# X1X1010/XequiNet

Hardware: AMD Instinct MI355X
Metric: edges/sec + achieved HBM GB/s, energy+force inference, QM9-shape batch (higher is better)
Workload: dtype f32

## Files before the change

include/xeq.h:

```cpp
#ifndef XEQ_H
#define XEQ_H
#include <stdint.h>

#ifdef __cplusplus
extern "C" {
#endif

enum { XEQ_F32 = 0, XEQ_F64 = 1 };
enum { XEQ_RBF_BESSEL = 0, XEQ_RBF_GAUSSIAN = 1, XEQ_RBF_EXPBERN = 2, XEQ_RBF_EXPNORM = 3 };
enum { XEQ_CUTOFF_COSINE = 0, XEQ_CUTOFF_POLYNOMIAL = 1 };
enum {
  XEQ_OK = 0,
  XEQ_ERR_INVALID_ARGUMENT = 1,
  XEQ_ERR_LAUNCH = 2,
  XEQ_ERR_UNSUPPORTED = 3
};

int xeq_version(void);
const char* xeq_last_error(void);
int64_t xeq_launch_count(void);
int64_t xeq_launch_names(int64_t first, char* buf, int64_t cap);


int xeq_csr_rowptr(const int64_t* keys, int64_t n_keys, int64_t n_rows, int32_t* rowptr, void* stream);
// ... 229 lines not shown
int xeq_message_q_wgrad(int dtype, const void* q, const void* basis, int64_t n_edges, int num_basis, int node_dim, const int32_t mul[3],
                        int n_chunks, void* parts, void* stream);

int xeq_message_wq_supported(int num_basis, int node_dim, const int32_t mul[3]);
int xeq_message_wq_fits(int64_t n_nodes, int64_t n_edges, int num_basis, int node_dim, const int32_t mul[3]);
int64_t xeq_message_wq_pcap(int64_t n_nodes, int64_t n_edges);
int xeq_message_wq_waves(void);
int xeq_message_wq_record_floats_for(int num_basis);
int xeq_message_wq_record_floats(void);
int64_t xeq_message_wq_plan_workspace(int64_t n_nodes);
int64_t xeq_message_wq_win_ints(int n_ranges);
int xeq_message_wq_plan(const int32_t* rowptr, const int32_t* perm, const int64_t* owner, const int64_t* gather,
                        int64_t n_nodes, int64_t n_edges, int n_ranges, void* workspace, int64_t workspace_bytes,
                        int32_t* qptr, int32_t* pgath, int32_t* peid, int32_t* qinfo, int32_t* sq, int32_t* sn, int32_t* win,
                        void* stream);
int xeq_edge_basis_wq(const void* vec, int64_t n_nodes, int64_t n_edges, const int32_t* qptr, const int32_t* peid,
                      int rbf_kind, int cutoff_kind, int num_basis, double cutoff, const void* p0, const void* p1,
                      void* basis, void* dbasis, void* stream);
int xeq_message_fwd_wq(int64_t n_nodes, int64_t n_edges, int n_ranges, const int32_t* sq, const int32_t* sn, const int32_t* win,
                       const int32_t* c_rowptr, const int32_t* pgath, const int32_t* qinfo, const void* basis, const void* h,
                       const void* xhat, const void* s_in, const void* x_in, const void* w_rbf, const void* b_rbf,
                       int num_basis, int node_dim, const int32_t mul[3], void* s_out, void* x_out, int xhat_layout,
                       void* stream);
int64_t xeq_message_wq_parts_floats(int64_t n_nodes, int64_t n_edges, const int32_t mul[3]);
#define XEQ_XHAT_HIGHER_L_ZERO 2
#define XEQ_WQ_MIRROR_WALK 4
#define XEQ_WQ_PACKED_WEIGHTS 64
int64_t xeq_message_wq_packed_weight_floats(int num_basis, int node_dim, const int32_t mul[3]);
int xeq_message_wq_pack_weights(const void* w_rbf, const void* b_rbf, int num_basis, int node_dim, const int32_t mul[3], void* packed,
                                void* stream);
// ... 49 lines not shown
                      int64_t n, int node_dim, const int32_t mul[3], int do_norm, const float* w_packed0, const float* w_packed1,
                      const float* w_packed2, int has_bias, double eps, float* cat, int64_t ld_cat, float* p, float* uv_bt,
                      float* stats, void* stream);
int xeq_update_uv_bwd(const float* uv_bt, const float* g_p, const float* g_cat, int64_t ld_cat, const float* g_x_out,
                      const float* g_s_out, const float* a, int64_t ld_a, const float* s, const float* x, const float* stats,
                      const float* ln_w, const float* eq_w, int64_t n, int node_dim, const int32_t mul[3], int do_norm,
                      const float* wt_packed0, const float* wt_packed1, const float* wt_packed2, double eps, float* g_s, float* g_x,
                      float* g_xhat_bt, void* stream);

long long xeq_pack_epoch(void);
void xeq_pack_epoch_bump(void);
int xeq_rowptr_guard(const int32_t* raw, int64_t n_nodes, int64_t capacity, int32_t* rowptr, int32_t* count, void* stream);
int xeq_rowptr_from_degrees(const int32_t* deg, int64_t n_nodes, int64_t capacity, int32_t* rowptr, int32_t* count, int64_t* running_total,
                            void* stream);
int64_t xeq_rowptr_from_degrees_max(void);

int xeq_node_block_supported(int dtype, int node_dim, const int32_t mul[3]);
int xeq_node_block_auto(int64_t n);
int64_t xeq_small_rows_limit(void);
int xeq_node_block_set_waves(int waves);
int64_t xeq_node_block_rows(int64_t n);
int64_t xeq_node_block_fwd_tiles(int with_tail);
int xeq_node_block_pack_fwd(const float* w3, const float* uv0, const float* uv1, const float* uv2, const float* dot, const float* w4,
                            const float* w1_next, const float* w2_next, void* out, void* stream);
int xeq_node_block_fwd(int64_t n, const float* s, const float* x, const float* ln_w, const float* ln_b, const float* eq_w, const float* eq_b,
                       const float* b_uv, const float* b3, const float* b4, double eps, const void* packed, float* p_scratch, float* uv_bt, float* stats,
                       float* pre, float* a, float* ip, float* s_out, float* x_out, const float* ln_w_next, const float* ln_b_next,
                       const float* eq_w_next, const float* eq_b_next, const float* b1_next, const float* b2_next, float* stats_next,
                       float* xhat_next, float* pre_next, float* h_next, void* stream);
int64_t xeq_node_block_bwd_tiles(int with_tail, int with_gx);
// ... 36 lines not shown
```

xequinet_amd/csrc/xeq_common.h:

```cpp
#pragma once
#include <hip/hip_runtime.h>
#include <stdint.h>
#include <stdlib.h>

#include "../../include/xeq.h"

namespace xeq {

void set_error(const char* fmt, ...);
void note_launch(const char* name);

#define XEQ_CHECK_ARG(cond, ...)        \
  do {                                  \
    if (!(cond)) {                      \
      xeq::set_error(__VA_ARGS__);      \
      return XEQ_ERR_INVALID_ARGUMENT;  \
    }                                   \
  } while (0)

#define XEQ_CHECK_LAUNCH(name)                                                   \
  do {                                                                           \
    xeq::note_launch(name);                                                      \
    hipError_t e_ = hipGetLastError();                                           \
    if (e_ != hipSuccess) {                                                      \
// ... 274 lines not shown
    aux[SCAN_WG_THREADS / 64] = run;
  }
  __syncthreads();
  int32_t base = aux[wave] + incl - sum;
  for (int64_t i = i0; i < i1; ++i) {
    const int32_t v = vals[i];
    vals[i] = base;
    base += v;
  }
  const int32_t total = aux[SCAN_WG_THREADS / 64];
  __syncthreads();
  return total;
}
inline size_t wg_scan_lds_bytes(int64_t n) { return sizeof(int32_t) * (size_t)(n + SCAN_WG_THREADS / 64 + 1); }

struct XcdWalk {
  int64_t n_items;
  int chunk;
  int label, slot, n_slots;
  int64_t idx;
  __device__ XcdWalk(int64_t n, int chunk_) : n_items(n), chunk(chunk_) {
    int nb = gridDim.x;
    if (nb >= 8) {
      label = blockIdx.x & 7;
      slot = blockIdx.x >> 3;
      n_slots = (nb - label + 7) >> 3;
    } else {
      label = -1;
      slot = blockIdx.x;
      n_slots = nb;
// ... 28 lines not shown
```

xequinet_amd/csrc/xeq_graph.hip:

```cpp
#include <stdarg.h>
#include <stdio.h>

#include <atomic>
#include <cmath>

#include <hipcub/hipcub.hpp>

#include "xeq_common.h"

namespace xeq {

static thread_local char g_err[512] = "";
void set_error(const char* fmt, ...) {
  va_list ap;
  va_start(ap, fmt);
  vsnprintf(g_err, sizeof(g_err), fmt, ap);
  va_end(ap);
}

static std::atomic<int64_t> g_launches{0};
constexpr int64_t LAUNCH_RING = 8192;
static const char* g_launch_ring[LAUNCH_RING];
void note_launch(const char* name) { g_launch_ring[g_launches.fetch_add(1, std::memory_order_relaxed) & (LAUNCH_RING - 1)] = name; }

// ... 565 lines not shown
__global__ void __launch_bounds__(SCAN_WG_THREADS) k_rowptr_from_degrees(const int32_t* __restrict__ deg, int64_t n, int64_t cap,
                                                                        int32_t* __restrict__ rowptr, int32_t* __restrict__ count,
                                                                        int64_t* __restrict__ running_total) {
  extern __shared__ int32_t scan_lds[];
  const int32_t total = wg_scan_lds([&](int64_t i) { return deg[i]; }, n, scan_lds);
  const bool ok = cap < 0 || (int64_t)total <= cap;
#pragma unroll 4
  for (int64_t i = threadIdx.x; i < n; i += SCAN_WG_THREADS) rowptr[i] = ok ? scan_lds[i] : 0;
  if (threadIdx.x == 0) {
    rowptr[n] = ok ? total : 0;
    if (count) count[0] = total;
    if (running_total) running_total[0] += total;
  }
}

__global__ void k_rowptr_guard(const int32_t* __restrict__ raw, int64_t n, int32_t cap, int32_t* __restrict__ rowptr, int32_t* __restrict__ count) {
  const int64_t i = (int64_t)blockIdx.x * blockDim.x + threadIdx.x;
  if (i > n) return;
  const int32_t total = raw[n];
  if (i == n) count[0] = total;
  rowptr[i] = total > cap ? 0 : raw[i];
}

}

using namespace xeq;

namespace xeq {
template <typename T>
struct CellGeom {
// ... 290 lines not shown
  XEQ_CHECK_ARG((deg || n_nodes == 0) && rowptr && n_nodes >= 0 && capacity < ((int64_t)1 << 31), "xeq_rowptr_from_degrees: bad arguments");
  if (n_nodes > SCAN_WG_MAX_ITEMS) {
    xeq::set_error("xeq_rowptr_from_degrees: %lld nodes (the one-workgroup form takes <= %lld)", (long long)n_nodes, (long long)SCAN_WG_MAX_ITEMS);
    return XEQ_ERR_UNSUPPORTED;
  }
  static const bool attr_ok = hipFuncSetAttribute((const void*)xeq::k_rowptr_from_degrees, hipFuncAttributeMaxDynamicSharedMemorySize,
                                                  (int)wg_scan_lds_bytes(SCAN_WG_MAX_ITEMS)) == hipSuccess;
  XEQ_CHECK_ARG(attr_ok, "xeq_rowptr_from_degrees: cannot reserve %zu bytes of LDS", wg_scan_lds_bytes(SCAN_WG_MAX_ITEMS));
  hipLaunchKernelGGL(xeq::k_rowptr_from_degrees, dim3(1), dim3(SCAN_WG_THREADS), wg_scan_lds_bytes(n_nodes), (hipStream_t)stream, deg, n_nodes,
                     capacity, rowptr, count, running_total);
  XEQ_CHECK_LAUNCH("xeq_rowptr_from_degrees");
  return XEQ_OK;
}
int64_t xeq_rowptr_from_degrees_max(void) { return SCAN_WG_MAX_ITEMS; }

int xeq_pbc_image_counts(int dtype, const void* cell_host, int64_t n_graphs, const int32_t pbc[3], double cutoff, int32_t reps[3]) {
  XEQ_CHECK_ARG(n_graphs >= 1 && cell_host != nullptr && cutoff > 0, "xeq_pbc_image_counts: bad arguments");
  if (dtype == XEQ_F32) xeq::image_counts<float>((const float*)cell_host, n_graphs, pbc, cutoff, reps);
  else if (dtype == XEQ_F64) xeq::image_counts<double>((const double*)cell_host, n_graphs, pbc, cutoff, reps);
  else XEQ_CHECK_ARG(false, "xeq_pbc_image_counts: dtype %d", dtype);
  XEQ_CHECK_ARG(reps[0] <= 64 && reps[1] <= 64 && reps[2] <= 64, "xeq_pbc_image_counts: %d x %d x %d images per axis (degenerate cell?)",
                (int)reps[0], (int)reps[1], (int)reps[2]);
  return XEQ_OK;
}

int xeq_pbc_tables_host(int dtype, const void* cell_host, int64_t n_graphs, const int32_t reps[3], double cutoff, void* out_host,
                        int64_t out_count) {
  XEQ_CHECK_ARG(n_graphs >= 1 && cell_host != nullptr && out_host != nullptr && reps[0] >= 0 && reps[1] >= 0 && reps[2] >= 0,
                "xeq_pbc_tables_host: bad arguments");
  const int64_t nc = (int64_t)(2 * reps[0] + 1) * (2 * reps[1] + 1) * (2 * reps[2] + 1);
// ... 195 lines not shown
```

xequinet_amd/csrc/xeq_message_wq.hip:

```cpp
#include "xeq_common.h"

#include <hipcub/hipcub.hpp>
#include <stdlib.h>

namespace xeq {

typedef float f32x16 __attribute__((ext_vector_type(16)));
typedef float f32x4 __attribute__((ext_vector_type(4)));
typedef int i32x4 __attribute__((ext_vector_type(4)));

typedef __bf16 bf16x8 __attribute__((ext_vector_type(8)));

constexpr bool wq_bftail(int ks) { return ks <= 3; }
constexpr int WQ_TAIL = 24;
constexpr int wq_tailw(int ks) { return ks <= 4 ? 4 : 8; }
constexpr int wq_recf(int ks) { return WQ_TAIL + 2 * wq_tailw(ks) + 8; }
constexpr int wq_yoff(int ks) { return WQ_TAIL + 2 * wq_tailw(ks); }
constexpr int wq_tail_values(int num_basis) { return (num_basis > 16 ? num_basis - 16 : 0) + 1; }
constexpr int wq_ks(int num_basis) {
  return wq_tail_values(num_basis) <= 1 ? 1 : (wq_tail_values(num_basis) <= 5 ? 3 : ((wq_tail_values(num_basis) + 1) / 2 < 4 ? 4 : (wq_tail_values(num_basis) + 1) / 2));
}
constexpr int WQ_REC_MAX = 48;
__device__ __forceinline__ uint32_t wq_bf16_rne(float x) {
  const uint32_t u = __float_as_uint(x);
  return (u + 0x7FFFu + ((u >> 16) & 1u)) >> 16;
}
__device__ __forceinline__ void wq_split3(float x, uint32_t& hi, uint32_t& mid, uint32_t& lo) {
  hi = wq_bf16_rne(x);
  const float r1 = x - __uint_as_float(hi << 16);
  mid = wq_bf16_rne(r1);
  const float r2 = r1 - __uint_as_float(mid << 16);
  lo = wq_bf16_rne(r2);
}
__device__ __forceinline__ int wq_tail_k(int q, int B) { return 16 + q < B ? 16 + q : (16 + q == (B > 16 ? B : 16) ? -1 : -2); }
constexpr uint32_t WQ_FIRST = 1u << 30, WQ_LAST = 1u << 31, WQ_OWNER = (1u << 30) - 1u;
#ifndef XEQ_WQ_WAVES
#define XEQ_WQ_WAVES 4
#endif
constexpr int WQ_WAVES = XEQ_WQ_WAVES;

#ifndef XEQ_WQ_PART_BWD
struct QuadCount {
  const int32_t* rowptr;
  int64_t n;
  __host__ __device__ int32_t operator()(int64_t i) const {
    if (i >= n) return 0;
    const int32_t deg = rowptr[i + 1] - rowptr[i];
    return deg > 0 ? (deg + 3) >> 2 : 1;
  }
};
#ifndef XEQ_WQ_PART_BWD
__global__ void __launch_bounds__(SCAN_WG_THREADS) k_wq_quad_scan(const QuadCount op, int32_t* __restrict__ qptr) {
  extern __shared__ int32_t scan_lds[];
  const int32_t total = wg_scan_lds(op, op.n, scan_lds);
#pragma unroll 4
  for (int64_t i = threadIdx.x; i < op.n; i += SCAN_WG_THREADS) qptr[i] = scan_lds[i];
  if (threadIdx.x == 0) qptr[op.n] = total;
}
#endif

__global__ void k_wq_fill(int64_t E, int64_t n_nodes, const int32_t* __restrict__ rowptr, const int32_t* __restrict__ perm,
                          const int64_t* __restrict__ owner, const int64_t* __restrict__ gather,
                          const int32_t* __restrict__ qptr, int32_t* __restrict__ pgath, int32_t* __restrict__ peid,
// ... 21 lines not shown
  if (k == deg - 1)
    for (int64_t pp = p + 1; pp < 4 * (int64_t)(q0 + nq); ++pp) {
      pgath[pp] = (int32_t)n;
      peid[pp] = -1;
    }
  if ((k & 3) == 0) {
    const int32_t g = k >> 2;
    qinfo[q0 + g] = (uint32_t)n | (g == 0 ? WQ_FIRST : 0u) | (g == nq - 1 ? WQ_LAST : 0u);
  }
}

__global__ void k_wq_streams(const int32_t* __restrict__ qptr, int64_t N, int n_ranges, int32_t* __restrict__ sq,
                             int32_t* __restrict__ sn) {
  const int k = blockIdx.x * blockDim.x + threadIdx.x;
  if (k > 2 * n_ranges) return;
  const int64_t Q = qptr[N];
  if (k == 2 * n_ranges) {
    sq[k] = (int32_t)Q;
    sn[k] = (int32_t)N;
    return;
  }
  const int64_t target = (int64_t)k * Q / (2 * n_ranges);
  int64_t lo = 0, hi = N;
  while (lo < hi) {
    const int64_t mid = (lo + hi) >> 1;
    if (qptr[mid] >= target) hi = mid;
    else lo = mid + 1;
  }
  sq[k] = qptr[lo];
  sn[k] = (int32_t)lo;
}

__global__ void k_wq_windows(const int32_t* __restrict__ sq, const int32_t* __restrict__ pgath, int n_ranges, int n_steps, int mult,
                             int32_t* __restrict__ win) {
  const int step = blockIdx.x, lane = threadIdx.x;
  if (step >= n_steps) return;
  const int k0 = min(2 * WQ_WAVES * mult * step, 2 * n_ranges), k1 = min(k0 + 2 * WQ_WAVES * mult, 2 * n_ranges);
  const int64_t p0 = 4 * (int64_t)sq[k0], p1 = 4 * (int64_t)sq[k1];
  int lo = 0x7fffffff, hi = -1;
  for (int64_t p = p0 + lane; p < p1; p += 64) {
    const int g = pgath[p];
    lo = g < lo ? g : lo;
    hi = g > hi ? g : hi;
  }
#pragma unroll
// ... 1546 lines not shown
    size_t temp = (size_t)workspace_bytes;
    if (hipcub::DeviceScan::ExclusiveSum(workspace, temp, it, qptr, (int)(n_nodes + 1), (hipStream_t)stream) != hipSuccess) {
      xeq::set_error("xeq_message_wq_plan: scan failed");
      return XEQ_ERR_LAUNCH;
    }
  }
  if (n_edges + n_nodes > 0) {
    hipLaunchKernelGGL(k_wq_fill, dim3((unsigned)((n_edges + n_nodes + 255) / 256)), dim3(256), 0, (hipStream_t)stream, n_edges, n_nodes,
                       rowptr, perm, owner, gather, (const int32_t*)qptr, pgath, peid, (uint32_t*)qinfo);
    XEQ_CHECK_LAUNCH("xeq_message_wq_plan (fill)");
  }
  const int n = 2 * n_ranges + 1;
  hipLaunchKernelGGL(k_wq_streams, dim3((unsigned)((n + 255) / 256)), dim3(256), 0, (hipStream_t)stream, (const int32_t*)qptr,
                     n_nodes, n_ranges, sq, sn);
  XEQ_CHECK_LAUNCH("xeq_message_wq_plan (streams)");
  const int n_steps = wq_class_steps(n_ranges, 1);
  hipLaunchKernelGGL(k_wq_windows, dim3((unsigned)n_steps), dim3(64), 0, (hipStream_t)stream, (const int32_t*)sq,
                     (const int32_t*)pgath, n_ranges, n_steps, 1, win);
  XEQ_CHECK_LAUNCH("xeq_message_wq_plan (windows)");
  const int mlong = wq_long_mult(n_edges, n_ranges);
  if (mlong > 1) {
    const int n_long = wq_class_steps(n_ranges, mlong);
    hipLaunchKernelGGL(k_wq_windows, dim3((unsigned)n_long), dim3(64), 0, (hipStream_t)stream, (const int32_t*)sq,
                       (const int32_t*)pgath, n_ranges, n_long, mlong, win + 2 * n_steps);
    XEQ_CHECK_LAUNCH("xeq_message_wq_plan (windows, long class)");
  }
  return XEQ_OK;
}

int64_t xeq_message_wq_win_ints(int n_ranges) {
  return 2 * ((int64_t)wq_class_steps(n_ranges, 1) + (int64_t)wq_class_steps(n_ranges, 2) + 1);
}

int xeq_edge_basis_wq(const void* vec, int64_t n_nodes, int64_t n_edges, const int32_t* qptr, const int32_t* peid,
                      int rbf_kind, int cutoff_kind, int num_basis, double cutoff, const void* p0, const void* p1,
                      void* basis, void* dbasis, void* stream) {
  XEQ_CHECK_ARG(n_edges >= 0 && n_nodes >= 0 && num_basis >= 1 && num_basis <= 31 && cutoff > 0, "xeq_edge_basis_wq: bad sizes");
  XEQ_CHECK_ARG(rbf_kind >= XEQ_RBF_BESSEL && rbf_kind <= XEQ_RBF_EXPNORM, "xeq_edge_basis_wq: rbf kernel %d is not implemented", rbf_kind);
  XEQ_CHECK_ARG(rbf_kind == XEQ_RBF_BESSEL || p1 != nullptr, "xeq_edge_basis_wq: this radial basis needs its second parameter array (std / logc / mu)");
// ... 166 lines not shown
```

xequinet_amd/lib.py:

```python
from __future__ import annotations

import ctypes
import os
from ctypes import c_char_p, c_double, c_int, c_int32, c_int64, c_void_p
from typing import Optional

import torch

_HERE = os.path.dirname(os.path.abspath(__file__))
LIB_PATH = os.environ.get("XEQ_LIB_PATH") or os.path.join(_HERE, "libxeq_hip.so")

XEQ_F32, XEQ_F64 = 0, 1
COPY_MANY_MAX = 16
SB_ACCUM_VEC = 16
XHAT_HIGHER_L_ZERO = 2
SB_Y0_ZERO = 8
SB_Q_ACCUMULATE = 16
SB_NO_GY = 32
WQ_MIRROR_WALK = 4
WQ_PACKED_WEIGHTS = 64
WQ_MAX_PART_SETS = 8
RBF_KINDS = {"bessel": 0, "gaussian": 1, "expbern": 2, "expnorm": 3}
CUTOFF_KINDS = {"cosine": 0, "polynomial": 1}

_P = c_void_p
# ... 39 lines not shown
    "xeq_eqln_bwd": [c_int, _P, _P, _P, c_int64, _I3, c_double, _P, _P],
    "xeq_segment_sum": [c_int, _P, _P, c_int64, c_int64, _P, _P],
    "xeq_linear_supported": [c_int, c_int, c_int],
    "xeq_mfma_order_probe": [_P, _P, _P, _P],
    "xeq_linear_fwd": [_P, c_int64, c_int64, c_int, _P, _P, c_int, c_int, c_int, _P, _P, c_int64, _P],
    "xeq_head_dot": [_P, c_int64, c_int, _P, _P, _P, _P],
    "xeq_head_bwd_hidden": [_P, c_int64, c_int, _P, _P, _P, _P],
    "xeq_head_supported": [c_int, c_int, c_int],
    "xeq_head_fwd": [_P, c_int64, c_int64, c_int, c_int, _P, _P, _P, _P, _P, _P, _P],
    "xeq_head_bwd": [_P, c_int64, c_int, _P, c_int64, _P, c_int64, _P, _P, _P],
    "xeq_electronic_supported": [c_int, c_int],
    "xeq_electronic_fwd": [c_int, _P, c_int64, c_int64, c_int, _P, c_int64, _P, _P, _P, _P, _P, _P, _P, _P, _P],
    "xeq_first_block_front": [_P, c_int, c_int64, c_int64, _P, _P, _P, c_int, c_int, c_int64, _P, _P, _P, _P],
    "xeq_rowptr_from_degrees": [_P, c_int64, c_int64, _P, _P, _P, _P],
    "xeq_rowptr_from_degrees_max": [],
    "xeq_wgrad_chunks": [c_int64, c_int, c_int],
    "xeq_wgrad": [_P, c_int64, _P, c_int64, c_int64, c_int, c_int, c_int, c_int, _P, _P],
    "xeq_load_padded_batch": [c_int, _P, _P, _P, _P, c_int64, c_int64, c_int64, c_int64, c_double, c_double, _P, _P, _P, _P, _P],
    "xeq_load_padded_batch_z64": [c_int, _P, _P, _P, _P, c_int64, c_int64, c_int64, c_int64, c_double, c_double, _P, _P, _P, _P, _P],
    "xeq_load_padded_shard": [c_int, _P, _P, c_int, _P, _P, c_int64, c_int64, c_int64, c_int64, c_int64, c_int64, c_double, c_double, _P, _P, _P, _P, _P],
    "xeq_copy_many": [c_int, ctypes.POINTER(c_void_p), ctypes.POINTER(c_void_p), ctypes.POINTER(c_int64), _P],
    "xeq_compare_many": [c_int, ctypes.POINTER(c_void_p), ctypes.POINTER(c_void_p), ctypes.POINTER(c_int64), ctypes.c_int32, _P, _P],
    "xeq_tensor_product_path": [c_int, _P, _P, c_int64, c_int, c_int, c_int, c_int, c_int, c_int, c_int, c_int, c_int, c_int, c_int,
                                c_int, c_int, _P, _P, c_int64, c_double, _P, _P],
    "xeq_tensor_product": [c_int, _P, _P, c_int64, c_int, c_int, c_int, c_int, ctypes.POINTER(ctypes.c_int32), _P, ctypes.POINTER(ctypes.c_int32),
                           c_int, _P, c_int64, ctypes.POINTER(ctypes.c_int32), ctypes.POINTER(c_double), _P, _P],
    "xeq_tensor_product_wgrad": [c_int, _P, _P, _P, c_int64, c_int, c_int, c_int, c_int, ctypes.POINTER(ctypes.c_int32), _P,
                                 ctypes.POINTER(ctypes.c_int32), ctypes.POINTER(ctypes.c_int32), ctypes.POINTER(ctypes.c_int32), c_int,
                                 ctypes.POINTER(c_double), c_int, _P, _P],
    "xeq_tensor_product_wgrad_chunks": [c_int64],
# ... 207 lines not shown
```

xequinet_amd/ops.py:

```python
from __future__ import annotations

import ctypes
from typing import Optional, Tuple

import torch
from torch.autograd import Function
from torch.autograd.function import once_differentiable

from . import lib
from .lib import call, dtype_code, mul3, ptr, require_hip, stream


class _KernelTimer:

    def __init__(self) -> None:
        self.enabled = False
        self.events = {}

    def reset(self, enabled: bool) -> None:
        self.enabled = enabled
        self.events = {}

    def launch(self, name: str, *args, label: Optional[str] = None) -> None:
        if not self.enabled:
# ... 108 lines not shown
            assert center_sorted and c_rowptr is not None
        if exact_mirror:
            rev = torch.empty(E, dtype=torch.int32, device=edge_index.device)
            call("xeq_reverse_edge_map", lib.ptr(edge_index), E, self.n_nodes, lib.ptr(self.c_rowptr), lib.ptr(rev), stream())
            self.mirror_map = rev
            self._n_view = (self.c_rowptr, rev)
        elif periodic_mirror:
            off = cell_offsets.contiguous()
            assert off.shape == (E, 3) and off.is_floating_point()
            rev = torch.empty(E, dtype=torch.int32, device=edge_index.device)
            call("xeq_reverse_edge_map_pbc", dtype_code(off), lib.ptr(edge_index), lib.ptr(off), E, self.n_nodes, lib.ptr(self.c_rowptr),
                 lib.ptr(rev), stream())
            self.mirror_map = rev
        else:
            self._sorted_neighbor_view()

    def _sorted_neighbor_view(self):
        if self._n_view is None:
            nbr = self.edge_index[1]
            if self._capacity_form:
                self._n_view = csr_by_key(nbr, self.n_nodes, n_valid=self.c_rowptr[self.n_nodes:])
            else:
                self._n_view = csr_by_key(nbr, self.n_nodes)
        return self._n_view

    @property
    def n_rowptr(self) -> torch.Tensor:
        return self._sorted_neighbor_view()[0]

    @property
# ... 113 lines not shown
    deg = torch.empty(N, dtype=torch.int32, device=dev)
    rowptr = torch.empty(N + 1, dtype=torch.int32, device=dev)
    dt = dtype_code(pos)
    call("xeq_radius_graph_count", dt, ptr(pos), ptr(ptr_), G, N, float(cutoff), ptr(deg), stream())
    count = torch.empty(1, dtype=torch.int32, device=dev)
    if N <= _scan_one_launch_max():
        call("xeq_rowptr_from_degrees", ptr(deg), N, cap, ptr(rowptr), ptr(count), ptr(running_total), stream())
    else:
        raw = torch.empty(N + 1, dtype=torch.int32, device=dev)
        _exclusive_scan(deg, N, raw)
        call("xeq_rowptr_guard", ptr(raw), N, cap, ptr(rowptr), ptr(count), stream())
        if running_total is not None:
            running_total.add_(count)
    call("xeq_radius_graph_fill", dt, ptr(pos), ptr(ptr_), G, N, float(cutoff), ptr(rowptr), cap, ptr(edge_index), stream())
    return rowptr, count


def radius_graph_pbc_raw(pos_wrap, ptr_, img, cells, shift, cutoff, prune=None):
    require_hip(pos_wrap, ptr_, img, cells, shift)
    pos_wrap, img, cells, shift = (t.contiguous() for t in (pos_wrap, img, cells, shift))
    if prune is not None and len(prune) == 4:
        recip, thr, reps, nbins = prune
        recip, thr = recip.to(pos_wrap.dtype).contiguous(), thr.to(pos_wrap.dtype).contiguous()
        nbins = nbins.to(torch.int32).contiguous()
        ptr_ = ptr_.to(torch.int64).contiguous()
        N, G, n_cells = pos_wrap.shape[0], ptr_.numel() - 1, cells.shape[0]
        dev, dt = pos_wrap.device, dtype_code(pos_wrap)
        per_graph = nbins.prod(dim=1)
        bin_base = torch.zeros(G + 1, dtype=torch.int32, device=dev)
        bin_base[1:] = torch.cumsum(per_graph, 0)
# ... 65 lines not shown
    _exclusive_scan(deg, N, rowptr)
    count = rowptr[N:].clone()
    rowptr.clamp_(max=cap)
    call("xeq_radius_graph_pbc_fill_pruned", dt, ptr(pos_wrap), ptr(ptr_), G, N, ptr(img), ptr(cells), ptr(shift), n_cells,
         float(cutoff), ptr(recip), ptr(thr), mul3(reps), ptr(rowptr), cap, ptr(edge_index), ptr(cell_offsets), stream())
    return rowptr, count


class EdgeVectors(Function):

    @staticmethod
    def forward(ctx, pos, graph: EdgeGraph, cell, cell_offsets, batch, strain=None, graph_ptr=None):
        require_hip(pos)
        pos_c = pos.contiguous()
        E = graph.n_edges
        vec = torch.empty((E, 3), dtype=pos.dtype, device=pos.device)
        dist = torch.empty((E,), dtype=pos.dtype, device=pos.device)
        cell, cell_offsets, batch = _c(cell), _c(cell_offsets), _c(batch)
        call("xeq_edge_vectors_fwd", dtype_code(pos), ptr(pos_c), ptr(graph.edge_index), E, ptr(cell), ptr(cell_offsets),
             ptr(batch), ptr(vec), ptr(dist), stream())
        graph._basis = None
        for plan in (graph._wq or {}).values():
            plan["records"] = None
        ctx.graph = graph
        ctx.graph_ptr = graph_ptr
        ctx.n_graphs = None if strain is None else strain.shape[0]
        ctx.save_for_backward(vec, dist)
        ctx.set_materialize_grads(False)
        return vec, dist

    @staticmethod
    @once_differentiable
    def backward(ctx, g_vec, g_dist):
        vec, dist = ctx.saved_tensors
        graph = ctx.graph
# ... 739 lines not shown
```

xequinet_amd/runtime.py:

```python
from __future__ import annotations

from collections import OrderedDict
from typing import Dict, Optional

import torch

from . import keys, lib, ops


class _Captured:
    def __init__(self) -> None:
        self.graph: Optional[torch.cuda.CUDAGraph] = None
        self.inputs: Dict[str, torch.Tensor] = {}
        self.edge_graph: Optional[ops.EdgeGraph] = None
        self.derived_batch = False
        self.outputs: Dict[str, torch.Tensor] = {}
        self.static: Dict[str, object] = {}
        self.graph_same: Optional[torch.cuda.CUDAGraph] = None
        self.outputs_same: Dict[str, torch.Tensor] = {}


def refuse_electronic(model, who: str) -> None:
    m = model
    while not isinstance(m, torch.nn.Module) and hasattr(m, "model"):
# ... 183 lines not shown
    mods = getattr(net, "mods", None)
    emb = mods["embedding"] if (mods is not None and "embedding" in mods) else None
    if emb is None or not hasattr(emb, "node_irreps"):
        return
    zero = getattr(step, "_zero_x", None)
    if zero is None:
        zero = step._zero_x = torch.zeros((step.n_atoms, emb.node_irreps.dim), dtype=step.pos.dtype, device=step.pos.device)
    data[ZERO_EQUIVARIANT] = zero


class GraphedStep:

    PAD_SPACING = 100.0

    def __init__(self, model: torch.nn.Module, capacity, cutoff: Optional[float] = None, compute_forces: bool = True, warmup: int = 2,
                 device=None, dtype=None) -> None:
        refuse_electronic(model, "GraphedStep")
        self.model = model
        self.n_atoms, self.n_graphs, self.n_edges = (int(c) for c in capacity)
        self.n_graphs += 1
        self.cutoff = float(model.cutoff_radius if cutoff is None else cutoff)
        self.compute_forces = compute_forces
        p = next(model.parameters())
        dev = p.device if device is None else torch.device(device)
        dt = p.dtype if dtype is None else dtype
        N, G, E = self.n_atoms, self.n_graphs, self.n_edges
        self.pos = torch.zeros((N, 3), dtype=dt, device=dev)
        self.z = torch.zeros(N, dtype=torch.int32, device=dev)
        self.ptr = torch.zeros(G + 1, dtype=torch.int64, device=dev)
        self.batch = torch.zeros(N, dtype=torch.int64, device=dev)
        self.edge_index = torch.zeros((2, max(E, 1)), dtype=torch.int64, device=dev)
        self.graph: Optional[torch.cuda.CUDAGraph] = None
        self.outputs: Dict[str, torch.Tensor] = {}
        self.rowptr: Optional[torch.Tensor] = None
        self.warmup = warmup
        self.captures = 0
        self._param_state = None
        self.edge_total = torch.zeros(1, dtype=torch.int64, device=self.pos.device)

    def overflowed(self) -> bool:
        return bool(self.outputs) and int(self.outputs["n_edges"].item()) > self.n_edges

    def _step(self) -> Dict[str, torch.Tensor]:
        rowptr, count = ops.radius_graph_capacity(self.pos, self.ptr, self.cutoff, self.edge_index, running_total=self.edge_total)
        eg = ops.EdgeGraph(self.edge_index, self.n_atoms, center_sorted=True, ptr=self.ptr, c_rowptr=rowptr, symmetric=True)
        data = {keys.POSITIONS: self.pos.detach(), keys.ATOMIC_NUMBERS: self.z, keys.EDGE_INDEX: self.edge_index, keys.BATCH: self.batch,
                keys.BATCH_PTR: self.ptr, keys.EDGE_GRAPH: eg}
        _offer_zero_start(self, data)
        with torch.enable_grad():
            out = self.model(data, compute_forces=self.compute_forces, compute_virial=False)
        res = {k: v.detach() for k, v in out.items() if isinstance(v, torch.Tensor)}
        res["n_edges"] = count
        return res

    def _load_shard(self, pos: torch.Tensor, atomic_numbers: torch.Tensor, ptr: torch.Tensor, batch: torch.Tensor, a: int, b: int, g0: int,
                    g1: int) -> None:
        from .lib import call, dtype_code
        from ctypes import c_void_p

        n, g = b - a, g1 - g0
# ... 512 lines not shown
```

Before: 181.0 million.

## Merge radius-graph fill with message work-quad plan and edge vectors

Adds a single-workgroup front scan that produces rowptr, quad pointers and stream boundaries together. It also adds a fill kernel that writes edge indices, edge vectors, distances, reverse map and the work-quad gather tables in one pass. The graphed step uses this merged path by default when every message layer picks the wq implementation, and the edge-vector op reuses the precomputed vectors. This removes separate plan, reverse-map and edge-vector kernels from the graph front, at the cost of an O(i) inner loop per hit for computing reverse indices.

```diff
diff --git a/include/xeq.h b/include/xeq.h
--- a/include/xeq.h
+++ b/include/xeq.h
@@ -267,6 +267,7 @@
                         int64_t n_nodes, int64_t n_edges, int n_ranges, void* workspace, int64_t workspace_bytes,
                         int32_t* qptr, int32_t* pgath, int32_t* peid, int32_t* qinfo, int32_t* sq, int32_t* sn, int32_t* win,
                         void* stream);
+int xeq_message_wq_windows(const int32_t* sq, const int32_t* pgath, int64_t n_edges, int n_ranges, int32_t* win, void* stream);
 int xeq_edge_basis_wq(const void* vec, int64_t n_nodes, int64_t n_edges, const int32_t* qptr, const int32_t* peid,
                       int rbf_kind, int cutoff_kind, int num_basis, double cutoff, const void* p0, const void* p1,
                       void* basis, void* dbasis, void* stream);
@@ -346,6 +347,11 @@
 int xeq_rowptr_from_degrees(const int32_t* deg, int64_t n_nodes, int64_t capacity, int32_t* rowptr, int32_t* count, int64_t* running_total,
                             void* stream);
 int64_t xeq_rowptr_from_degrees_max(void);
+int xeq_front_scan(const int32_t* deg, int64_t n_nodes, int64_t capacity, int n_ranges, int32_t* rowptr, int32_t* count,
+                   int64_t* running_total, int32_t* qptr, int32_t* sq, int32_t* sn, void* stream);
+int xeq_radius_graph_fill_plan(int dtype, const void* pos, const int64_t* ptr, int64_t n_graphs, int64_t n_nodes, double cutoff,
+                               const int32_t* rowptr, const int32_t* count, int64_t n_edges, const int32_t* qptr, int64_t* edge_index,
+                               void* vec, void* dist, int32_t* rev, int32_t* pgath, int32_t* peid, int32_t* qinfo, void* stream);
 
 int xeq_node_block_supported(int dtype, int node_dim, const int32_t mul[3]);
 int xeq_node_block_auto(int64_t n);
diff --git a/xequinet_amd/csrc/xeq_common.h b/xequinet_amd/csrc/xeq_common.h
--- a/xequinet_amd/csrc/xeq_common.h
+++ b/xequinet_amd/csrc/xeq_common.h
@@ -312,6 +312,27 @@
 }
 inline size_t wg_scan_lds_bytes(int64_t n) { return sizeof(int32_t) * (size_t)(n + SCAN_WG_THREADS / 64 + 1); }
 
+__host__ __device__ __forceinline__ int32_t wq_quads_of_degree(int32_t deg) { return deg > 0 ? (deg + 3) >> 2 : 1; }
+constexpr uint32_t WQ_FIRST = 1u << 30, WQ_LAST = 1u << 31, WQ_OWNER = (1u << 30) - 1u;
+template <typename QP>
+__device__ __forceinline__ void wq_stream_boundary(const QP& qptr, int64_t N, int64_t Q, int k, int n_ranges, int32_t* __restrict__ sq,
+                                                   int32_t* __restrict__ sn) {
+  if (k == 2 * n_ranges) {
+    sq[k] = (int32_t)Q;
+    sn[k] = (int32_t)N;
+    return;
+  }
+  const int64_t target = (int64_t)k * Q / (2 * n_ranges);
+  int64_t lo = 0, hi = N;
+  while (lo < hi) {
+    const int64_t mid = (lo + hi) >> 1;
+    if (qptr(mid) >= target) hi = mid;
+    else lo = mid + 1;
+  }
+  sq[k] = qptr(lo);
+  sn[k] = (int32_t)lo;
+}
+
 struct XcdWalk {
   int64_t n_items;
   int chunk;
diff --git a/xequinet_amd/csrc/xeq_graph.hip b/xequinet_amd/csrc/xeq_graph.hip
--- a/xequinet_amd/csrc/xeq_graph.hip
+++ b/xequinet_amd/csrc/xeq_graph.hip
@@ -603,6 +603,101 @@
   }
 }
 
+__global__ void __launch_bounds__(SCAN_WG_THREADS) k_front_scan(const int32_t* __restrict__ deg, int64_t n, int64_t cap, int n_ranges,
+                                                               int32_t* __restrict__ rowptr, int32_t* __restrict__ count,
+                                                               int64_t* __restrict__ running_total, int32_t* __restrict__ qptr,
+                                                               int32_t* __restrict__ sq, int32_t* __restrict__ sn) {
+  extern __shared__ int32_t scan_lds[];
+  const int32_t total = wg_scan_lds([&](int64_t i) { return deg[i]; }, n, scan_lds);
+  const bool ok = cap < 0 || (int64_t)total <= cap;
+#pragma unroll 4
+  for (int64_t i = threadIdx.x; i < n; i += SCAN_WG_THREADS) rowptr[i] = ok ? scan_lds[i] : 0;
+  if (threadIdx.x == 0) {
+    rowptr[n] = ok ? total : 0;
+    if (count) count[0] = total;
+    if (running_total) running_total[0] += total;
+  }
+  __syncthreads();
+  const int32_t quads = wg_scan_lds([&](int64_t i) { return wq_quads_of_degree(ok ? deg[i] : 0); }, n, scan_lds);
+#pragma unroll 4
+  for (int64_t i = threadIdx.x; i < n; i += SCAN_WG_THREADS) qptr[i] = scan_lds[i];
+  if (threadIdx.x == 0) qptr[n] = quads;
+  for (int k = threadIdx.x; k <= 2 * n_ranges; k += SCAN_WG_THREADS)
+    wq_stream_boundary([&](int64_t m) { return m < n ? scan_lds[m] : quads; }, n, quads, k, n_ranges, sq, sn);
+}
+
+template <typename T> __device__ __forceinline__ T edge_length(T v0, T v1, T v2);
+template <> __device__ __forceinline__ float edge_length<float>(float v0, float v1, float v2) {
+  return sqrt_<float>(__fmaf_rn(v2, v2, __fmaf_rn(v0, v0, __fmul_rn(v1, v1))));
+}
+template <> __device__ __forceinline__ double edge_length<double>(double v0, double v1, double v2) {
+  return sqrt_<double>(__fma_rn(v2, v2, __fma_rn(v0, v0, __dmul_rn(v1, v1))));
+}
+
+template <typename T>
+__global__ void k_radius_graph_fill_plan(const T* __restrict__ pos, const int64_t* __restrict__ ptr, int64_t n_graphs, int64_t n_nodes, T r2,
+                                         const int32_t* __restrict__ rowptr, const int32_t* __restrict__ count, int64_t n_edges,
+                                         const int32_t* __restrict__ qptr, int64_t* __restrict__ edge_index, T* __restrict__ vec,
+                                         T* __restrict__ dist, int32_t* __restrict__ rev, int32_t* __restrict__ pgath,
+                                         int32_t* __restrict__ peid, uint32_t* __restrict__ qinfo) {
+  const int lane = threadIdx.x & 63;
+  const int64_t i = ((int64_t)blockIdx.x * blockDim.x + threadIdx.x) >> 6;
+  if (i >= n_nodes) return;
+  const bool fits = (int64_t)count[0] <= n_edges;
+  const int64_t q0 = qptr[i];
+  int32_t deg = 0;
+  if (fits) {
+    const int64_t g = graph_of(ptr, n_graphs, i);
+    const int64_t a = ptr[g], b = ptr[g + 1];
+    const T xi = pos[3 * i], yi = pos[3 * i + 1], zi = pos[3 * i + 2];
+    const int64_t r0 = rowptr[i];
+    int64_t w = r0;
+    for (int64_t j0 = a; j0 < b; j0 += 64) {
+      const int64_t j = j0 + lane;
+      bool hit = false;
+      T xj = T(0), yj = T(0), zj = T(0), dx = T(0), dy = T(0), dz = T(0);
+      if (j < b) {
+        xj = pos[3 * j], yj = pos[3 * j + 1], zj = pos[3 * j + 2];
+        dx = sub_rn<T>(xi, xj), dy = sub_rn<T>(yi, yj), dz = sub_rn<T>(zi, zj);
+        T d2 = add_rn<T>(add_rn<T>(mul_rn<T>(dx, dx), mul_rn<T>(dy, dy)), mul_rn<T>(dz, dz));
+        hit = d2 < r2 && j != i;
+      }
+      const unsigned long long m = __ballot(hit);
+      if (m != 0ull) {
+        int32_t below = 0;
+        for (int64_t k = a; k < i; ++k) {
+          const T ex = sub_rn<T>(xj, pos[3 * k]), ey = sub_rn<T>(yj, pos[3 * k + 1]), ez = sub_rn<T>(zj, pos[3 * k + 2]);
+          const T e2 = add_rn<T>(add_rn<T>(mul_rn<T>(ex, ex), mul_rn<T>(ey, ey)), mul_rn<T>(ez, ez));
+          below += (e2 < r2 && k != j) ? 1 : 0;
+        }
+        if (hit) {
+          const int64_t p = w + __popcll(m & ((1ull << lane) - 1ull));
+          if (p < n_edges) {
+            edge_index[p] = i;
+            edge_index[n_edges + p] = j;
+            vec[3 * p] = dx;
+            vec[3 * p + 1] = dy;
+            vec[3 * p + 2] = dz;
+            if (dist) dist[p] = edge_length<T>(dx, dy, dz);
+            rev[p] = rowptr[j] + below;
+            const int64_t s = 4 * q0 + (p - r0);
+            pgath[s] = (int32_t)j;
+            peid[s] = (int32_t)p;
+          }
+        }
+      }
+      w += __popcll(m);
+    }
+    deg = (int32_t)(w - r0);
+  }
+  const int32_t nq = wq_quads_of_degree(deg);
+  if (lane < 4 * nq - deg) {
+    pgath[4 * q0 + deg + lane] = (int32_t)i;
+    peid[4 * q0 + deg + lane] = -1;
+  }
+  for (int32_t q = lane; q < nq; q += 64) qinfo[q0 + q] = (uint32_t)i | (q == 0 ? WQ_FIRST : 0u) | (q == nq - 1 ? WQ_LAST : 0u);
+}
+
 __global__ void k_rowptr_guard(const int32_t* __restrict__ raw, int64_t n, int32_t cap, int32_t* __restrict__ rowptr, int32_t* __restrict__ count) {
   const int64_t i = (int64_t)blockIdx.x * blockDim.x + threadIdx.x;
   if (i > n) return;
@@ -923,6 +1018,42 @@
 }
 int64_t xeq_rowptr_from_degrees_max(void) { return SCAN_WG_MAX_ITEMS; }
 
+int xeq_front_scan(const int32_t* deg, int64_t n_nodes, int64_t capacity, int n_ranges, int32_t* rowptr, int32_t* count,
+                   int64_t* running_total, int32_t* qptr, int32_t* sq, int32_t* sn, void* stream) {
+  XEQ_CHECK_ARG((deg || n_nodes == 0) && rowptr && qptr && sq && sn && n_nodes >= 0 && n_ranges >= 1 && capacity < ((int64_t)1 << 31),
+                "xeq_front_scan: bad arguments");
+  if (n_nodes > SCAN_WG_MAX_ITEMS) {
+    xeq::set_error("xeq_front_scan: %lld nodes (the one-workgroup form takes <= %lld)", (long long)n_nodes, (long long)SCAN_WG_MAX_ITEMS);
+    return XEQ_ERR_UNSUPPORTED;
+  }
+  static const bool attr_ok = hipFuncSetAttribute((const void*)xeq::k_front_scan, hipFuncAttributeMaxDynamicSharedMemorySize,
+                                                  (int)wg_scan_lds_bytes(SCAN_WG_MAX_ITEMS)) == hipSuccess;
+  XEQ_CHECK_ARG(attr_ok, "xeq_front_scan: cannot reserve %zu bytes of LDS", wg_scan_lds_bytes(SCAN_WG_MAX_ITEMS));
+  hipLaunchKernelGGL(xeq::k_front_scan, dim3(1), dim3(SCAN_WG_THREADS), wg_scan_lds_bytes(n_nodes), (hipStream_t)stream, deg, n_nodes,
+                     capacity, n_ranges, rowptr, count, running_total, qptr, sq, sn);
+  XEQ_CHECK_LAUNCH("xeq_front_scan");
+  return XEQ_OK;
+}
+
+int xeq_radius_graph_fill_plan(int dtype, const void* pos, const int64_t* ptr, int64_t n_graphs, int64_t n_nodes, double cutoff,
+                               const int32_t* rowptr, const int32_t* count, int64_t n_edges, const int32_t* qptr, int64_t* edge_index,
+                               void* vec, void* dist, int32_t* rev, int32_t* pgath, int32_t* peid, int32_t* qinfo, void* stream) {
+  XEQ_CHECK_ARG(n_graphs >= 0 && n_nodes >= 0 && n_edges >= 0 && n_edges < ((int64_t)1 << 31) && n_nodes < ((int64_t)1 << 30),
+                "xeq_radius_graph_fill_plan: bad sizes");
+  if (n_nodes == 0) return XEQ_OK;
+  XEQ_CHECK_ARG(n_graphs > 0, "xeq_radius_graph_fill_plan: nodes without graphs");
+  XEQ_CHECK_ARG(pos && ptr && rowptr && count && qptr && edge_index && vec && rev && pgath && peid && qinfo,
+                "xeq_radius_graph_fill_plan: NULL argument");
+  XEQ_DISPATCH_FLOAT(dtype, {
+    T rc = (T)cutoff;
+    hipLaunchKernelGGL((k_radius_graph_fill_plan<T>), dim3((unsigned)((n_nodes + 3) / 4)), dim3(256), 0, (hipStream_t)stream,
+                       (const T*)pos, ptr, n_graphs, n_nodes, rc * rc, rowptr, count, n_edges, qptr, edge_index, (T*)vec, (T*)dist, rev,
+                       pgath, peid, (uint32_t*)qinfo);
+  });
+  XEQ_CHECK_LAUNCH("xeq_radius_graph_fill_plan");
+  return XEQ_OK;
+}
+
 int xeq_pbc_image_counts(int dtype, const void* cell_host, int64_t n_graphs, const int32_t pbc[3], double cutoff, int32_t reps[3]) {
   XEQ_CHECK_ARG(n_graphs >= 1 && cell_host != nullptr && cutoff > 0, "xeq_pbc_image_counts: bad arguments");
   if (dtype == XEQ_F32) xeq::image_counts<float>((const float*)cell_host, n_graphs, pbc, cutoff, reps);
diff --git a/xequinet_amd/csrc/xeq_message_wq.hip b/xequinet_amd/csrc/xeq_message_wq.hip
--- a/xequinet_amd/csrc/xeq_message_wq.hip
+++ b/xequinet_amd/csrc/xeq_message_wq.hip
@@ -33,7 +33,6 @@
   lo = wq_bf16_rne(r2);
 }
 __device__ __forceinline__ int wq_tail_k(int q, int B) { return 16 + q < B ? 16 + q : (16 + q == (B > 16 ? B : 16) ? -1 : -2); }
-constexpr uint32_t WQ_FIRST = 1u << 30, WQ_LAST = 1u << 31, WQ_OWNER = (1u << 30) - 1u;
 #ifndef XEQ_WQ_WAVES
 #define XEQ_WQ_WAVES 4
 #endif
@@ -45,8 +44,7 @@
   int64_t n;
   __host__ __device__ int32_t operator()(int64_t i) const {
     if (i >= n) return 0;
-    const int32_t deg = rowptr[i + 1] - rowptr[i];
-    return deg > 0 ? (deg + 3) >> 2 : 1;
+    return wq_quads_of_degree(rowptr[i + 1] - rowptr[i]);
   }
 };
 #ifndef XEQ_WQ_PART_BWD
@@ -98,21 +96,7 @@
                              int32_t* __restrict__ sn) {
   const int k = blockIdx.x * blockDim.x + threadIdx.x;
   if (k > 2 * n_ranges) return;
-  const int64_t Q = qptr[N];
-  if (k == 2 * n_ranges) {
-    sq[k] = (int32_t)Q;
-    sn[k] = (int32_t)N;
-    return;
-  }
-  const int64_t target = (int64_t)k * Q / (2 * n_ranges);
-  int64_t lo = 0, hi = N;
-  while (lo < hi) {
-    const int64_t mid = (lo + hi) >> 1;
-    if (qptr[mid] >= target) hi = mid;
-    else lo = mid + 1;
-  }
-  sq[k] = qptr[lo];
-  sn[k] = (int32_t)lo;
+  wq_stream_boundary([&](int64_t m) { return qptr[m]; }, N, qptr[N], k, n_ranges, sq, sn);
 }
 
 __global__ void k_wq_windows(const int32_t* __restrict__ sq, const int32_t* __restrict__ pgath, int n_ranges, int n_steps, int mult,
@@ -1689,15 +1673,19 @@
   hipLaunchKernelGGL(k_wq_streams, dim3((unsigned)((n + 255) / 256)), dim3(256), 0, (hipStream_t)stream, (const int32_t*)qptr,
                      n_nodes, n_ranges, sq, sn);
   XEQ_CHECK_LAUNCH("xeq_message_wq_plan (streams)");
+  return xeq_message_wq_windows(sq, pgath, n_edges, n_ranges, win, stream);
+}
+
+int xeq_message_wq_windows(const int32_t* sq, const int32_t* pgath, int64_t n_edges, int n_ranges, int32_t* win, void* stream) {
+  XEQ_CHECK_ARG(sq && pgath && win && n_edges >= 0 && n_ranges >= 1, "xeq_message_wq_windows: bad arguments");
   const int n_steps = wq_class_steps(n_ranges, 1);
-  hipLaunchKernelGGL(k_wq_windows, dim3((unsigned)n_steps), dim3(64), 0, (hipStream_t)stream, (const int32_t*)sq,
-                     (const int32_t*)pgath, n_ranges, n_steps, 1, win);
+  hipLaunchKernelGGL(k_wq_windows, dim3((unsigned)n_steps), dim3(64), 0, (hipStream_t)stream, sq, pgath, n_ranges, n_steps, 1, win);
   XEQ_CHECK_LAUNCH("xeq_message_wq_plan (windows)");
   const int mlong = wq_long_mult(n_edges, n_ranges);
   if (mlong > 1) {
     const int n_long = wq_class_steps(n_ranges, mlong);
-    hipLaunchKernelGGL(k_wq_windows, dim3((unsigned)n_long), dim3(64), 0, (hipStream_t)stream, (const int32_t*)sq,
-                       (const int32_t*)pgath, n_ranges, n_long, mlong, win + 2 * n_steps);
+    hipLaunchKernelGGL(k_wq_windows, dim3((unsigned)n_long), dim3(64), 0, (hipStream_t)stream, sq, pgath, n_ranges, n_long, mlong,
+                       win + 2 * n_steps);
     XEQ_CHECK_LAUNCH("xeq_message_wq_plan (windows, long class)");
   }
   return XEQ_OK;
diff --git a/xequinet_amd/lib.py b/xequinet_amd/lib.py
--- a/xequinet_amd/lib.py
+++ b/xequinet_amd/lib.py
@@ -9,6 +9,8 @@
 
 _HERE = os.path.dirname(os.path.abspath(__file__))
 LIB_PATH = os.environ.get("XEQ_LIB_PATH") or os.path.join(_HERE, "libxeq_hip.so")
+
+FRONT_MERGED = os.environ.get("XEQ_FRONT_SEPARATE", "0") in ("", "0")
 
 XEQ_F32, XEQ_F64 = 0, 1
 COPY_MANY_MAX = 16
@@ -78,6 +80,9 @@
     "xeq_first_block_front": [_P, c_int, c_int64, c_int64, _P, _P, _P, c_int, c_int, c_int64, _P, _P, _P, _P],
     "xeq_rowptr_from_degrees": [_P, c_int64, c_int64, _P, _P, _P, _P],
     "xeq_rowptr_from_degrees_max": [],
+    "xeq_front_scan": [_P, c_int64, c_int64, c_int, _P, _P, _P, _P, _P, _P, _P],
+    "xeq_radius_graph_fill_plan": [c_int, _P, _P, c_int64, c_int64, c_double, _P, _P, c_int64, _P, _P, _P, _P, _P, _P, _P, _P, _P],
+    "xeq_message_wq_windows": [_P, _P, c_int64, c_int, _P, _P],
     "xeq_wgrad_chunks": [c_int64, c_int, c_int],
     "xeq_wgrad": [_P, c_int64, _P, c_int64, c_int64, c_int, c_int, c_int, c_int, _P, _P],
     "xeq_load_padded_batch": [c_int, _P, _P, _P, _P, c_int64, c_int64, c_int64, c_int64, c_double, c_double, _P, _P, _P, _P, _P],
diff --git a/xequinet_amd/ops.py b/xequinet_amd/ops.py
--- a/xequinet_amd/ops.py
+++ b/xequinet_amd/ops.py
@@ -146,6 +146,20 @@
             self.mirror_map = rev
         else:
             self._sorted_neighbor_view()
+
+    @classmethod
+    def prebuilt(cls, edge_index: torch.Tensor, n_nodes: int, ptr: Optional[torch.Tensor], c_rowptr: torch.Tensor, mirror_map: torch.Tensor,
+                 plan_key, plan, vec: torch.Tensor, dist: torch.Tensor, pos: torch.Tensor) -> "EdgeGraph":
+        g = cls.__new__(cls)
+        g.ptr, g._wq, g._basis = ptr, {plan_key: plan}, None
+        g.edge_index, g.n_nodes, g.n_edges = edge_index, int(n_nodes), int(edge_index.shape[1])
+        g.c_perm, g.c_rowptr = None, c_rowptr
+        g.mirror_walk, g.periodic, g.cell_offsets = True, False, None
+        g.mirror_map = mirror_map
+        g.edge_count_on_device, g._capacity_form = False, False
+        g._n_view = (c_rowptr, mirror_map)
+        g._edge_vectors = (pos.data_ptr(), vec, dist)
+        return g
 
     def _sorted_neighbor_view(self):
         if self._n_view is None:
@@ -289,6 +303,34 @@
             running_total.add_(count)
     call("xeq_radius_graph_fill", dt, ptr(pos), ptr(ptr_), G, N, float(cutoff), ptr(rowptr), cap, ptr(edge_index), stream())
     return rowptr, count
+
+
+def radius_graph_capacity_plan(pos: torch.Tensor, ptr_: torch.Tensor, cutoff: float, edge_index: torch.Tensor,
+                               running_total: Optional[torch.Tensor] = None):
+    require_hip(pos, ptr_, edge_index)
+    pos = pos.detach().contiguous()
+    ptr_ = ptr_.to(torch.int64).contiguous()
+    assert edge_index.dim() == 2 and edge_index.shape[0] == 2 and edge_index.dtype == torch.int64 and edge_index.is_contiguous()
+    N, G, cap = pos.shape[0], ptr_.numel() - 1, int(edge_index.shape[1])
+    assert pos.dtype == torch.float32 and 0 < N <= _scan_one_launch_max()
+    dev, dt, L = pos.device, dtype_code(pos), lib.load()
+    eps = _wq_edges_per_stream(cap, N)
+    n_ranges = max(1, -(-cap // (2 * eps)))
+    pcap = int(L.xeq_message_wq_pcap(N, cap))
+    i32 = lambda n: torch.empty(max(int(n), 1), dtype=torch.int32, device=dev)
+    deg, rowptr, count, rev = i32(N), i32(N + 1), i32(1), i32(cap)
+    plan = {"reverse": False, "n_ranges": n_ranges, "pcap": pcap, "qptr": i32(N + 1), "pgath": i32(pcap), "peid": i32(pcap),
+            "qinfo": i32(pcap // 4), "sq": i32(2 * n_ranges + 1), "sn": i32(2 * n_ranges + 1),
+            "win": i32(int(L.xeq_message_wq_win_ints(n_ranges))), "work": None, "records": None, "rowptr": rowptr}
+    vec = torch.empty((cap, 3), dtype=pos.dtype, device=dev)
+    dist = torch.empty((cap,), dtype=pos.dtype, device=dev)
+    call("xeq_radius_graph_count", dt, ptr(pos), ptr(ptr_), G, N, float(cutoff), ptr(deg), stream())
+    call("xeq_front_scan", ptr(deg), N, cap, n_ranges, ptr(rowptr), ptr(count), ptr(running_total), ptr(plan["qptr"]), ptr(plan["sq"]),
+         ptr(plan["sn"]), stream())
+    call("xeq_radius_graph_fill_plan", dt, ptr(pos), ptr(ptr_), G, N, float(cutoff), ptr(rowptr), ptr(count), cap, ptr(plan["qptr"]),
+         ptr(edge_index), ptr(vec), ptr(dist), ptr(rev), ptr(plan["pgath"]), ptr(plan["peid"]), ptr(plan["qinfo"]), stream())
+    call("xeq_message_wq_windows", ptr(plan["sq"]), ptr(plan["pgath"]), cap, n_ranges, ptr(plan["win"]), stream())
+    return EdgeGraph.prebuilt(edge_index, N, ptr_, rowptr, rev, (False, int(eps)), plan, vec, dist, pos), count
 
 
 def radius_graph_pbc_raw(pos_wrap, ptr_, img, cells, shift, cutoff, prune=None):
@@ -384,11 +426,15 @@
         require_hip(pos)
         pos_c = pos.contiguous()
         E = graph.n_edges
-        vec = torch.empty((E, 3), dtype=pos.dtype, device=pos.device)
-        dist = torch.empty((E,), dtype=pos.dtype, device=pos.device)
-        cell, cell_offsets, batch = _c(cell), _c(cell_offsets), _c(batch)
-        call("xeq_edge_vectors_fwd", dtype_code(pos), ptr(pos_c), ptr(graph.edge_index), E, ptr(cell), ptr(cell_offsets),
-             ptr(batch), ptr(vec), ptr(dist), stream())
+        ready, graph._edge_vectors = getattr(graph, "_edge_vectors", None), None
+        if ready is not None and cell is None and ready[0] == pos_c.data_ptr():
+            vec, dist = ready[1], ready[2]
+        else:
+            vec = torch.empty((E, 3), dtype=pos.dtype, device=pos.device)
+            dist = torch.empty((E,), dtype=pos.dtype, device=pos.device)
+            cell, cell_offsets, batch = _c(cell), _c(cell_offsets), _c(batch)
+            call("xeq_edge_vectors_fwd", dtype_code(pos), ptr(pos_c), ptr(graph.edge_index), E, ptr(cell), ptr(cell_offsets),
+                 ptr(batch), ptr(vec), ptr(dist), stream())
         graph._basis = None
         for plan in (graph._wq or {}).values():
             plan["records"] = None
diff --git a/xequinet_amd/runtime.py b/xequinet_amd/runtime.py
--- a/xequinet_amd/runtime.py
+++ b/xequinet_amd/runtime.py
@@ -221,7 +221,7 @@
     PAD_SPACING = 100.0
 
     def __init__(self, model: torch.nn.Module, capacity, cutoff: Optional[float] = None, compute_forces: bool = True, warmup: int = 2,
-                 device=None, dtype=None) -> None:
+                 device=None, dtype=None, merged_front: Optional[bool] = None) -> None:
         refuse_electronic(model, "GraphedStep")
         self.model = model
         self.n_atoms, self.n_graphs, self.n_edges = (int(c) for c in capacity)
@@ -244,13 +244,28 @@
         self.captures = 0
         self._param_state = None
         self.edge_total = torch.zeros(1, dtype=torch.int64, device=self.pos.device)
+        self.merged_front = (lib.FRONT_MERGED if merged_front is None else bool(merged_front)) and self._takes_merged_front()
+
+    def _takes_merged_front(self) -> bool:
+        from .nn.xpainn import XPainnMessage
+
+        net = self.model
+        while not isinstance(net, torch.nn.Module) and hasattr(net, "model"):
+            net = net.model
+        msgs = [m for m in net.modules() if isinstance(m, XPainnMessage)] if isinstance(net, torch.nn.Module) else []
+        if not msgs or self.pos.dtype != torch.float32 or not self.pos.is_cuda or not 0 < self.n_atoms <= ops._scan_one_launch_max():
+            return False
+        return all(ops.select_message_impl(self.pos.dtype, self.n_atoms, max(self.n_edges, 1), m.num_basis, m.node_dim, m._mul) == "wq" for m in msgs)
 
     def overflowed(self) -> bool:
         return bool(self.outputs) and int(self.outputs["n_edges"].item()) > self.n_edges
 
     def _step(self) -> Dict[str, torch.Tensor]:
-        rowptr, count = ops.radius_graph_capacity(self.pos, self.ptr, self.cutoff, self.edge_index, running_total=self.edge_total)
-        eg = ops.EdgeGraph(self.edge_index, self.n_atoms, center_sorted=True, ptr=self.ptr, c_rowptr=rowptr, symmetric=True)
+        if self.merged_front:
+            eg, count = ops.radius_graph_capacity_plan(self.pos, self.ptr, self.cutoff, self.edge_index, running_total=self.edge_total)
+        else:
+            rowptr, count = ops.radius_graph_capacity(self.pos, self.ptr, self.cutoff, self.edge_index, running_total=self.edge_total)
+            eg = ops.EdgeGraph(self.edge_index, self.n_atoms, center_sorted=True, ptr=self.ptr, c_rowptr=rowptr, symmetric=True)
         data = {keys.POSITIONS: self.pos.detach(), keys.ATOMIC_NUMBERS: self.z, keys.EDGE_INDEX: self.edge_index, keys.BATCH: self.batch,
                 keys.BATCH_PTR: self.ptr, keys.EDGE_GRAPH: eg}
         _offer_zero_start(self, data)
```

After: 180.7 million, median of 2. Within noise of the previous version (-0.2%).
